# DeepMETv2/DeepMETv2

Hardware: AMD Instinct MI355X
Metric: events/sec (4.5k PF cands, k=16) (higher is better)
Workload: dtype f32

## Files before the change

### deepmetv2_amd/build.py

```python
from __future__ import annotations

import concurrent.futures as cf
import os
import shutil
import subprocess
import sys

PKG_DIR = os.path.dirname(os.path.abspath(__file__))
CSRC = os.path.join(PKG_DIR, "csrc")
OBJ_DIR = os.path.join(CSRC, "_obj")
LIB_PATH = os.path.join(PKG_DIR, "libdmet_hip.so")
SOURCES = ["knn.hip", "radius.hip", "edgeconv.hip", "edgemlp.hip", "misc.hip", "dense.hip", "encoder.hip", "norm.hip", "edgeconv_bwd.hip",
           "head.hip", "finalize.hip", "pool.hip",
           "edgemlp_f32.hip", "edgemlp_bf16.hip", "edgeconv_sum.hip", "gravnet.hip", "attention.hip", "fps.hip"]
HEADERS = [os.path.join(CSRC, h) for h in ("common.h", "knn_common.h", "knn_filter.h", "nls_body.h", "edgemlp_fused.h")] + \
          [os.path.join(PKG_DIR, "..", "include", "dmet.h")]
ARCH = "gfx950"
CXXFLAGS = ["-O3", "-std=c++17", "-fPIC", f"--offload-arch={ARCH}", "-ffp-contract=off", "-Wall",
            "-Wno-unused-function", "-DNDEBUG"]


def _hipcc() -> str:
    exe = shutil.which("hipcc") or "/opt/rocm/bin/hipcc"
    if not os.path.exists(exe):
        raise RuntimeError("hipcc not found: cannot build libdmet_hip.so")
    return exe


def _stale(target: str, deps) -> bool:
    if not os.path.exists(target):
        return True
    t = os.path.getmtime(target)
    return any(os.path.getmtime(d) > t for d in deps if os.path.exists(d))


def _compile(src: str, force: bool) -> str:
    obj = os.path.join(OBJ_DIR, os.path.splitext(src)[0] + ".o")
    path = os.path.join(CSRC, src)
    if force or _stale(obj, [path] + HEADERS):
        cmd = [_hipcc()] + CXXFLAGS + ["-c", path, "-o", obj]
        subprocess.check_call(cmd)
    return obj


def build_hip(force: bool = False, verbose: bool = False) -> str:
    os.makedirs(OBJ_DIR, exist_ok=True)
    with cf.ThreadPoolExecutor(max_workers=min(4, len(SOURCES))) as ex:
        objs = list(ex.map(lambda s: _compile(s, force), SOURCES))
    if force or _stale(LIB_PATH, objs):
        cmd = [_hipcc(), "-shared", "-fPIC", f"--offload-arch={ARCH}", "-o", LIB_PATH] + objs
        if verbose:
            print(" ".join(cmd))
        subprocess.check_call(cmd)
    return LIB_PATH


if __name__ == "__main__":
    print(build_hip(force="--force" in sys.argv, verbose=True))
```

### deepmetv2_amd/csrc/knn.hip

```cpp
#include <stdlib.h>

#include "common.h"
#include "knn_common.h"
#include "nls_body.h"

namespace dmet {
namespace {

constexpr int kTileC = 32;
constexpr int kQMax = 8;
constexpr int kMaxSplit = 8;
constexpr int kWavesPerGroup = 4;

#define DMET_PKSUB_LO " op_sel:[0,0] op_sel_hi:[0,1] neg_lo:[0,1] neg_hi:[0,1]\n\t"
#define DMET_PKSUB_HI " op_sel:[1,0] op_sel_hi:[1,1] neg_lo:[0,1] neg_hi:[0,1]\n\t"
__device__ __forceinline__ void pk_dist_step4(f2 &accA, f2 &accB, f2 vxy, f2 vzw, f2 wxy, f2 wzw, f2 q0, f2 q1, f2 q2,
                                              f2 q3)
{
    f2 t0, t1, t2, t3;
    asm("v_pk_add_f32 %[t0], %[vxy], %[q0]" DMET_PKSUB_LO
        "v_pk_add_f32 %[t1], %[wxy], %[q0]" DMET_PKSUB_LO
        "v_pk_add_f32 %[t2], %[vxy], %[q1]" DMET_PKSUB_HI
        "v_pk_add_f32 %[t3], %[wxy], %[q1]" DMET_PKSUB_HI
        "v_pk_fma_f32 %[a], %[t0], %[t0], %[a]\n\t"
        "v_pk_fma_f32 %[b], %[t1], %[t1], %[b]\n\t"
        "v_pk_add_f32 %[t0], %[vzw], %[q2]" DMET_PKSUB_LO
        "v_pk_add_f32 %[t1], %[wzw], %[q2]" DMET_PKSUB_LO
        "v_pk_fma_f32 %[a], %[t2], %[t2], %[a]\n\t"
        "v_pk_fma_f32 %[b], %[t3], %[t3], %[b]\n\t"
        "v_pk_add_f32 %[t2], %[vzw], %[q3]" DMET_PKSUB_HI
        "v_pk_add_f32 %[t3], %[wzw], %[q3]" DMET_PKSUB_HI
        "v_pk_fma_f32 %[a], %[t0], %[t0], %[a]\n\t"
        "v_pk_fma_f32 %[b], %[t1], %[t1], %[b]\n\t"
        "v_pk_fma_f32 %[a], %[t2], %[t2], %[a]\n\t"
        "v_pk_fma_f32 %[b], %[t3], %[t3], %[b]"
        : [a] "+v"(accA), [b] "+v"(accB), [t0] "=&v"(t0), [t1] "=&v"(t1), [t2] "=&v"(t2), [t3] "=&v"(t3)
        : [vxy] "v"(vxy), [vzw] "v"(vzw), [wxy] "v"(wxy), [wzw] "v"(wzw), [q0] "v"(q0), [q1] "v"(q1), [q2] "v"(q2),
          [q3] "v"(q3));
}

template <bool HI>
__device__ __forceinline__ void pk_sub2(f2 &tA, f2 &tB, f2 v, f2 w, f2 q)
{
    if (HI)
        asm("v_pk_add_f32 %[ta], %[v], %[q]" DMET_PKSUB_HI "v_pk_add_f32 %[tb], %[w], %[q]" DMET_PKSUB_HI
            : [ta] "=&v"(tA), [tb] "=&v"(tB) : [v] "v"(v), [w] "v"(w), [q] "v"(q));
    else
        asm("v_pk_add_f32 %[ta], %[v], %[q]" DMET_PKSUB_LO "v_pk_add_f32 %[tb], %[w], %[q]" DMET_PKSUB_LO
            : [ta] "=&v"(tA), [tb] "=&v"(tB) : [v] "v"(v), [w] "v"(w), [q] "v"(q));
}

__device__ __forceinline__ void pk_fma2(f2 &accA, f2 &accB, f2 tA, f2 tB)
{
    asm("v_pk_fma_f32 %[a], %[ta], %[ta], %[a]\n\t"
        "v_pk_fma_f32 %[b], %[tb], %[tb], %[b]"
        : [a] "+v"(accA), [b] "+v"(accB) : [ta] "v"(tA), [tb] "v"(tB));
}

__device__ __forceinline__ float wrap1(float d, float L)
{
    float a, t;
    asm("v_sub_f32 %[t], %[L], |%[d]|\n\t"
        "v_min_f32 %[a], |%[d]|, %[t]"
        : [a] "=v"(a), [t] "=&v"(t) : [d] "v"(d), [L] "s"(L));
    return a;
}

template <bool HI>
__device__ __forceinline__ void pk_dist_step1_per(f2 &accA, f2 &accB, f2 v, f2 w, f2 q, float L, bool wrap)
{
    f2 tA, tB;
    pk_sub2<HI>(tA, tB, v, w, q);
    if (wrap) {
        tA = f2{wrap1(tA.x, L), wrap1(tA.y, L)};
        tB = f2{wrap1(tB.x, L), wrap1(tB.y, L)};
    }
    pk_fma2(accA, accB, tA, tB);
}

template <int DP, int TQ>
struct KnnShared {
    float4 tile[(kTileC + 1) * DP / 4];
    uint2 queue[TQ][kQMax][kWave];
};

template <int KP>
__device__ __attribute__((noinline)) float drain_queue(const uint2 (*queue)[kWave], int lane, int cnt, bool fresh,
                                                       bool valid, float *__restrict__ ld,
                                                       int32_t *__restrict__ lj)
{
    float d[KP];
    int32_t j[KP];
    if (fresh || !valid) {
#pragma unroll
        for (int p = 0; p < KP; ++p) { d[p] = kKnnSentinel; j[p] = -1; }
    } else {
#pragma unroll
        for (int p = 0; p < KP; p += 4) {
            const float4 v = *reinterpret_cast<const float4 *>(ld + p);
            const int4 w = *reinterpret_cast<const int4 *>(lj + p);
            d[p] = v.x; d[p + 1] = v.y; d[p + 2] = v.z; d[p + 3] = v.w;
            j[p] = w.x; j[p + 1] = w.y; j[p + 2] = w.z; j[p + 3] = w.w;
        }
    }
    int maxcnt = cnt;
#pragma unroll
    for (int off = 32; off > 0; off >>= 1) maxcnt = max(maxcnt, __shfl_xor(maxcnt, off, 64));
    for (int s = 0; s < maxcnt; ++s) {
        if (s < cnt) {
            const uint2 e = queue[s][lane];
            const float nd = __uint_as_float(e.x);
            const int32_t nj = (int32_t)e.y;
            if (nd < d[KP - 1]) {
#pragma unroll
                for (int p = KP - 1; p >= 1; --p) {
                    const bool mq = d[p - 1] > nd;
                    const bool mp = d[p] > nd;
                    const float dn = mq ? d[p - 1] : (mp ? nd : d[p]);
                    const int32_t jn = mq ? j[p - 1] : (mp ? nj : j[p]);
                    d[p] = dn;
                    j[p] = jn;
                }
                if (d[0] > nd) { d[0] = nd; j[0] = nj; }
            }
        }
    }
    if (valid) {
#pragma unroll
        for (int p = 0; p < KP; p += 4) {
            *reinterpret_cast<float4 *>(ld + p) = make_float4(d[p], d[p + 1], d[p + 2], d[p + 3]);
            *reinterpret_cast<int4 *>(lj + p) = make_int4(j[p], j[p + 1], j[p + 2], j[p + 3]);
        }
    }
    return d[KP - 1];
}

#ifdef DMET_KNN_STAMP
__device__ unsigned long long g_knn_stamps[1 << 16][4];
#endif

#ifndef DMET_F2_MIN_NODES
#define DMET_F2_MIN_NODES 800
#endif
constexpr int kF2MinNodes = DMET_F2_MIN_NODES;
constexpr int kFilterMaxSplit = 2;
#ifndef DMET_F2_SPLIT_MIN_NODES
#define DMET_F2_SPLIT_MIN_NODES 2560
#endif
constexpr int kF2SplitMinNodes = DMET_F2_SPLIT_MIN_NODES;
constexpr int kF2MaxNodes = 65536;

struct KnnPlan {
    int total_tiles;
    int n_full;
    int split;
    int form1_events;
// ... 1118 lines not shown
```

### deepmetv2_amd/csrc/knn_filter.h

```cpp
constexpr int kFQ = 64;

typedef float f32x16 __attribute__((ext_vector_type(16)));
typedef short bf16x8 __attribute__((ext_vector_type(8)));
typedef _Float16 f16x8 __attribute__((ext_vector_type(8)));

struct KnnFilterArgs {
    const float *x;
    const int64_t *ptr;
    int B;
    int64_t N;
    int k;
    float *nrm;
    uint8_t *rec;
    const KnnPlan *plan;
    const int32_t *order;
    const int32_t *pos_of;
    const int32_t *tile_ptr;
    float *psd;
    int32_t *psj;
    int32_t *nbr;
    float *dist;
    uint16_t *nbr16;
    int32_t *flags;
    int32_t *any;
// ... 914 lines not shown
        asm volatile("" : "+v"(fq[0]), "+v"(fq[1]));
    }
    float rc = L.rep, rn;
    f32x16 c0 = f2_block<NH>(A, bq[0], fq[0]);
    f32x16 c1 = f2_block<NH>(A, bq[1], fq[1]);
    f32x16 n0, n1;
    f2_load<NH>(A, rec, rbase + min(t_lo + 1, t_hi - 1), lane, hh, rofs);
    float carry = kKnnSentinel;
    if constexpr (NH == 1 && UPD && REC) {
        F2Ops<NH> C;
        f2_load<NH>(B, rec, rbase + min(t_lo + 2, t_hi - 1), lane, hh, rofs);
        for (int t = t_lo; t < t_hi; t += 6) {
            f2_tile<M, UPD, REC, true, NH, false, 3>(L, S, rec, rbase, t, t_hi, c0, c1, n0, n1, rc, rn, A, C, bq, fq, lane, hh,
                                                     alive, carry, rofs);
            if (t + 1 >= t_hi) break;
            f2_tile<M, UPD, REC, true, NH, true, 3>(L, S, rec, rbase, t + 1, t_hi, n0, n1, c0, c1, rn, rc, B, A, bq, fq, lane,
                                                    hh, alive, carry, rofs);
            if (t + 2 >= t_hi) break;
            f2_tile<M, UPD, REC, true, NH, false, 3>(L, S, rec, rbase, t + 2, t_hi, c0, c1, n0, n1, rc, rn, C, B, bq, fq, lane,
                                                     hh, alive, carry, rofs);
            if (t + 3 >= t_hi) break;
            f2_tile<M, UPD, REC, true, NH, true, 3>(L, S, rec, rbase, t + 3, t_hi, n0, n1, c0, c1, rn, rc, A, C, bq, fq, lane,
                                                    hh, alive, carry, rofs);
            if (t + 4 >= t_hi) break;
            f2_tile<M, UPD, REC, true, NH, false, 3>(L, S, rec, rbase, t + 4, t_hi, c0, c1, n0, n1, rc, rn, B, A, bq, fq, lane,
                                                     hh, alive, carry, rofs);
            if (t + 5 >= t_hi) break;
            f2_tile<M, UPD, REC, true, NH, true, 3>(L, S, rec, rbase, t + 5, t_hi, n0, n1, c0, c1, rn, rc, C, B, bq, fq, lane,
                                                    hh, alive, carry, rofs);
        }
        return;
    }
    for (int t = t_lo; t < t_hi; t += 2) {
        f2_tile<M, UPD, REC, true, NH, false>(L, S, rec, rbase, t, t_hi, c0, c1, n0, n1, rc, rn, A, B, bq, fq, lane, hh, alive,
                                              carry, rofs);
        if (t + 1 < t_hi)
            f2_tile<M, UPD, REC, true, NH, true>(L, S, rec, rbase, t + 1, t_hi, n0, n1, c0, c1, rn, rc, B, A, bq, fq, lane, hh,
                                                 alive, carry, rofs);
    }
}

__device__ __forceinline__ int filter_group(const KnnFilterArgs &a)
{
    const int full_groups = a.plan->n_full / kWavesPerGroup;
    return (int)blockIdx.x < full_groups ? xcd_swizzle((int)blockIdx.x, full_groups) : (int)blockIdx.x;
}

template <int KP, int NH = 1>
__device__ __forceinline__ void filter2_wave(const KnnFilterArgs &a, F2Wave &S, int *tickets, int group, int wv, int lane)
{
    constexpr int M = f2_list_len(KP);
    constexpr int D = 32 * NH;
    constexpr int MS = (M + 1 + 3) & ~3;
    const int col = lane & 31, hh = lane >> 5;
    const uint8_t *__restrict__ rec = a.rec;
    const int64_t *__restrict__ ptr = a.ptr;

    const int n_full = a.plan->n_full, split = a.plan->split, total = a.plan->total_tiles;
    const int item = group * kWavesPerGroup + wv;
    int tile = item, sub = 0, nsub = 1;
    if (item >= n_full) {
        const int r = item - n_full;
        tile = n_full + r / split;
        sub = r % split;
        nsub = split;
    }
    if (tile >= total) return;
    const int pos = find_tile_event(a.tile_ptr, a.B, tile);
    const int ev = a.order[pos];
    const int ev_lo = (int)ptr[ev], ev_hi = (int)ptr[ev + 1];
    const int q_first = ev_lo + (tile - a.tile_ptr[pos]) * kFQ;
    if (!f2_in_domain(ev_hi - ev_lo)) {
        if (NH != 1 && sub == 0) {
            const int q = q_first + lane;
            if (q < ev_hi) {
                flag_query(a, q, a.xtile_ptr[pos] + (q - ev_lo) / a.xtile_queries);
            }
        }
        return;
    }
    int clo = ev_lo, chi = ev_hi;
    if (nsub > 1) {
        if (ev_hi - ev_lo < kF2SplitMinNodes) {
            if (sub != 0) return;
            nsub = 1;
        } else {
            const int chunk = (((chi - clo) + nsub - 1) / nsub + 31) & ~31;
            clo = min(chi, clo + sub * chunk);
            chi = min(chi, clo + chunk);
        }
    }
    const int64_t rbase = (ptr[ev] >> 5) + ev;
    const int64_t rlast = rbase + (ev_hi - ev_lo - 1) / 32;
    const int t_lo = (clo - ev_lo) / 32, t_hi = (chi - ev_lo + 31) / 32;

    const int myq = q_first + hh * 32 + col;
    const bool valid = myq < ev_hi;
    float t_fix = -__builtin_inff();
    bool act = valid;
    for (int attempt = 0;; ++attempt) {
    F2Lane<M> L;
#pragma unroll
    for (int p = 0; p < M; ++p) L.tk[p] = kKnnSentinel;
    L.tau = attempt == 0 ? -__builtin_inff() : t_fix;
    L.tq = 0u;
    L.rep = 0.0f;
    L.cnt = 0;
    L.overflow = false;
    {
        f16x8 bq[2][2 * NH];
#pragma unroll
        for (int b = 0; b < 2; ++b) {
            const int64_t qrec = min(rbase + (q_first - ev_lo) / 32 + b, rlast);
            const f16x8 *g = reinterpret_cast<const f16x8 *>(rec + qrec * rec_bytes(NH));
#pragma unroll
            for (int m = 0; m < 2 * NH; ++m) bq[b][m] = g[m * 64 + lane] * (_Float16)-2.0f;
        }
        if (attempt == 0) {
            const int t_def = min(t_hi, t_lo + kF2Defer);
            f2_sweep<M, true, false, NH>(L, S, rec, rbase, t_lo, t_def, bq, lane, hh, valid);
            f2_sweep<M, true, true, NH>(L, S, rec, rbase, t_def, t_hi, bq, lane, hh, valid);
            if (a.cut_scale >= 0.0f) {
                float tkk = kKnnSentinel;
#pragma unroll
                for (int p = 0; p < KP; ++p)
                    if (p == a.k - 1) tkk = L.tk[p];
                if (tkk < kKnnSentinel) {
                    int qi = valid ? myq : ev_lo;
                    asm volatile("" : "+v"(qi));
                    const float cut = f2_cut<NH>(tkk, a.nrm[qi], a.cut_scale);
                    L.tau = fminf(L.tau, cut);
                }
            }
            f2_sweep<M, false, true, NH>(L, S, rec, rbase, t_lo, t_def, bq, lane, hh, valid);
        } else {
            f2_sweep<M, false, true, NH>(L, S, rec, rbase, t_lo, t_hi, bq, lane, hh, valid);
        }
    }
    f2_compact<M>(L, S, lane, kF2Slots);
#if defined(DMET_F2_ABL) && DMET_F2_ABL >= 1
    return;
#endif

    const int64_t qrow_id = valid ? myq : ev_lo;
    float qrow[D];
    {
        const float4 *g = reinterpret_cast<const float4 *>(a.x + qrow_id * D);
#pragma unroll
        for (int c = 0; c < D / 4; ++c) {
            const float4 v = g[c];
            qrow[4 * c] = v.x; qrow[4 * c + 1] = v.y; qrow[4 * c + 2] = v.z; qrow[4 * c + 3] = v.w;
        }
    }
    unsigned long long kk[KP];
#pragma unroll
    for (int p = 0; p < KP; ++p) kk[p] = (unsigned long long)__float_as_uint(kKnnSentinel) << 32;
    const int nent = (act && !L.overflow) ? L.cnt : 0;
    int slot = 0;
    unsigned cmask = 0u;
    int ctile = 0;
    auto pop = [&]() __attribute__((always_inline)) -> int32_t {
        if (cmask == 0u && slot < nent) {
            const uint2 e = S.ent[slot][lane];
            cmask = e.x;
            ctile = (int)(e.y & kF2TileMask);
            ++slot;
        }
        int32_t j = -1;
        if (cmask != 0u) {
            const int r = __builtin_clz(cmask);
            cmask &= ~(0x80000000u >> r);
            j = ev_lo + ctile * 32 + f2_mask_row(r);
        }
        return j;
    };
    const float4 *x4 = reinterpret_cast<const float4 *>(a.x);
#ifdef DMET_RR_PRIO
    __builtin_amdgcn_s_setprio(DMET_RR_PRIO);
#endif
    if constexpr (NH != 1) {
        for (;;) {
            const int32_t j = pop();
            if (!__any(j >= 0)) break;
            const float4 *row = x4 + (int64_t)(j >= 0 ? j : ev_lo) * (D / 4);
            float4 v[D / 4];
#pragma unroll
            for (int c = 0; c < D / 4; ++c) v[c] = row[c];
            float dc = 0.0f;
#pragma unroll
            for (int c = 0; c < D / 4; ++c) {
                float df;
                df = v[c].x - qrow[4 * c + 0]; dc = __builtin_fmaf(df, df, dc);
                df = v[c].y - qrow[4 * c + 1]; dc = __builtin_fmaf(df, df, dc);
                df = v[c].z - qrow[4 * c + 2]; dc = __builtin_fmaf(df, df, dc);
                df = v[c].w - qrow[4 * c + 3]; dc = __builtin_fmaf(df, df, dc);
            }
            const unsigned long long nk =
                j >= 0 ? (((unsigned long long)__float_as_uint(dc) << 32) | (unsigned)j) : ~0ull;
            bool g[KP];
#pragma unroll
            for (int p = 0; p < KP; ++p) g[p] = kk[p] > nk;
#pragma unroll
            for (int p = KP - 1; p >= 1; --p) kk[p] = g[p - 1] ? kk[p - 1] : (g[p] ? nk : kk[p]);
            kk[0] = g[0] ? nk : kk[0];
        }
    } else {
    struct HalfRows { float4 v0, v1, v2, v3, v4, v5, v6, v7; };
#ifdef DMET_RR_FULLROW
    auto fetch = [&](int32_t j) __attribute__((always_inline)) -> HalfRows {
        const int32_t jc = j >= 0 ? j : ev_lo;
        const int64_t o = lane & 7;
        const int sub = lane >> 3;
        HalfRows R;
        R.v0 = x4[(int64_t)__shfl(jc, 0 + sub, 64) * 8 + o];
        R.v1 = x4[(int64_t)__shfl(jc, 8 + sub, 64) * 8 + o];
        R.v2 = x4[(int64_t)__shfl(jc, 16 + sub, 64) * 8 + o];
        R.v3 = x4[(int64_t)__shfl(jc, 24 + sub, 64) * 8 + o];
        R.v4 = x4[(int64_t)__shfl(jc, 32 + sub, 64) * 8 + o];
        R.v5 = x4[(int64_t)__shfl(jc, 40 + sub, 64) * 8 + o];
        R.v6 = x4[(int64_t)__shfl(jc, 48 + sub, 64) * 8 + o];
        R.v7 = x4[(int64_t)__shfl(jc, 56 + sub, 64) * 8 + o];
        return R;
    };
#else
    auto fetch = [&](int32_t j) __attribute__((always_inline)) -> HalfRows {
        const int32_t jc = j >= 0 ? j : ev_lo;
        const int64_t o = 4 * 0 + (lane & 3);
        const int64_t r0 = (int64_t)__shfl(jc, 0 + (lane >> 2), 64) * 8 + o;
        const int64_t r1 = (int64_t)__shfl(jc, 16 + (lane >> 2), 64) * 8 + o;
        const int64_t r2 = (int64_t)__shfl(jc, 32 + (lane >> 2), 64) * 8 + o;
        const int64_t r3 = (int64_t)__shfl(jc, 48 + (lane >> 2), 64) * 8 + o;
        HalfRows R;
        R.v0 = x4[r0]; R.v1 = x4[r1]; R.v2 = x4[r2]; R.v3 = x4[r3];
        R.v4 = x4[r0 + 4]; R.v5 = x4[r1 + 4]; R.v6 = x4[r2 + 4]; R.v7 = x4[r3 + 4];
        return R;
    };
#endif
    auto chain16 = [&](float dc, int h) __attribute__((always_inline)) -> float {
#pragma unroll
        for (int c4 = 0; c4 < 4; ++c4) {
            const float4 v = *reinterpret_cast<const float4 *>(&S.rows[lane][4 * c4]);
            const int f0 = 16 * h + 4 * c4;
            float df;
            df = v.x - qrow[f0 + 0]; dc = __builtin_fmaf(df, df, dc);
            df = v.y - qrow[f0 + 1]; dc = __builtin_fmaf(df, df, dc);
            df = v.z - qrow[f0 + 2]; dc = __builtin_fmaf(df, df, dc);
            df = v.w - qrow[f0 + 3]; dc = __builtin_fmaf(df, df, dc);
        }
        return dc;
    };
    auto round = [&](const HalfRows &R, int32_t j) __attribute__((always_inline)) {
#ifdef DMET_RR_FULLROW
        float4 *dst = reinterpret_cast<float4 *>(&S.rows[lane >> 3][4 * (lane & 3)]);
        constexpr int kS8 = 8 * (kF2RowF + 4) / 4;
        const bool lowhalf = (lane & 4) == 0;
        wave_sync();
        if (lowhalf) {
            dst[0] = R.v0; dst[kS8] = R.v1; dst[2 * kS8] = R.v2; dst[3 * kS8] = R.v3;
            dst[4 * kS8] = R.v4; dst[5 * kS8] = R.v5; dst[6 * kS8] = R.v6; dst[7 * kS8] = R.v7;
        }
        wave_sync();
        float dc = chain16(0.0f, 0);
        wave_sync();
        if (!lowhalf) {
            dst[0] = R.v0; dst[kS8] = R.v1; dst[2 * kS8] = R.v2; dst[3 * kS8] = R.v3;
            dst[4 * kS8] = R.v4; dst[5 * kS8] = R.v5; dst[6 * kS8] = R.v6; dst[7 * kS8] = R.v7;
        }
        wave_sync();
        dc = chain16(dc, 1);
#else
        float4 *dst = reinterpret_cast<float4 *>(&S.rows[lane >> 2][4 * (lane & 3)]);
        constexpr int kStride = 16 * (kF2RowF + 4) / 4;
        wave_sync();
        dst[0] = R.v0; dst[kStride] = R.v1; dst[2 * kStride] = R.v2; dst[3 * kStride] = R.v3;
        wave_sync();
        float dc = chain16(0.0f, 0);
        wave_sync();
        dst[0] = R.v4; dst[kStride] = R.v5; dst[2 * kStride] = R.v6; dst[3 * kStride] = R.v7;
        wave_sync();
        dc = chain16(dc, 1);
#endif
        const unsigned long long nk =
            j >= 0 ? (((unsigned long long)__float_as_uint(dc) << 32) | (unsigned)j) : ~0ull;
        bool g[KP];
#pragma unroll
        for (int p = 0; p < KP; ++p) g[p] = kk[p] > nk;
#pragma unroll
        for (int p = KP - 1; p >= 1; --p) kk[p] = g[p - 1] ? kk[p - 1] : (g[p] ? nk : kk[p]);
        kk[0] = g[0] ? nk : kk[0];
    };
#ifdef DMET_RR_THREE
    constexpr bool kThreeRounds = KP <= 16;
#else
    constexpr bool kThreeRounds = false;
#endif
    if constexpr (kThreeRounds) {
        int32_t ja = pop(), jb, jc;
        HalfRows pa = fetch(ja), pb, pc;
        jb = pop();
        pb = fetch(jb);
        for (;;) {
            if (!__any(ja >= 0)) break;
            jc = pop(); pc = fetch(jc);
            round(pa, ja);
            if (!__any(jb >= 0)) break;
            ja = pop(); pa = fetch(ja);
            round(pb, jb);
            if (!__any(jc >= 0)) break;
            jb = pop(); pb = fetch(jb);
            round(pc, jc);
        }
    } else {
        int32_t ja = pop(), jb;
        HalfRows pa = fetch(ja), pb;
        for (;;) {
            if (!__any(ja >= 0)) break;
            jb = pop(); pb = fetch(jb);
            round(pa, ja);
            if (!__any(jb >= 0)) break;
            ja = pop(); pa = fetch(ja);
            round(pb, jb);
        }
    }
    }
#ifdef DMET_RR_PRIO
    __builtin_amdgcn_s_setprio(0);
#endif
    float kd[KP];
    int32_t kj[KP];
#pragma unroll
    for (int p = 0; p < KP; ++p) {
        kd[p] = __uint_as_float((unsigned)(kk[p] >> 32));
        kj[p] = kd[p] == kKnnSentinel ? -1 : (int32_t)(unsigned)kk[p];
    }
    int elane = lane, eq = myq;
    asm volatile("" : "+v"(elane), "+v"(eq));
    const int k = a.k;
    const float tau = L.tau;
    auto emit = [&](const bool rows_on, const bool coop) __attribute__((always_inline)) -> float {
        float kth = -1.0f;
#pragma unroll
        for (int p = 0; p < KP; ++p)
            if (p == k - 1 && kj[p] >= 0) kth = kd[p];
        if constexpr (KP % 4 == 0 && KP <= 20) {
            if (coop && a.emit_coalesced && k == KP) {
                constexpr int RP = KP / 4;
                const unsigned long long on = __ballot(rows_on);
                unsigned *stg = reinterpret_cast<unsigned *>(&S);
                const int64_t blk = (int64_t)q_first * KP;
                wave_sync();
#pragma unroll
                for (int q = 0; q < RP; ++q)
                    *reinterpret_cast<uint4 *>(stg + elane * KP + 4 * q) =
                        make_uint4((unsigned)kj[4 * q], (unsigned)kj[4 * q + 1], (unsigned)kj[4 * q + 2], (unsigned)kj[4 * q + 3]);
                wave_sync();
#pragma unroll
                for (int t = 0; t < RP; ++t) {
                    const int pi = t * 64 + elane;
                    const uint4 v = *reinterpret_cast<const uint4 *>(stg + 4 * pi);
                    if ((on >> (pi / RP)) & 1ull) *reinterpret_cast<uint4 *>(a.nbr + blk + 4 * pi) = v;
                }
                wave_sync();
#pragma unroll
                for (int q = 0; q < RP; ++q)
                    *reinterpret_cast<uint4 *>(stg + elane * KP + 4 * q) =
                        make_uint4(__float_as_uint(kd[4 * q]), __float_as_uint(kd[4 * q + 1]), __float_as_uint(kd[4 * q + 2]),
                                   __float_as_uint(kd[4 * q + 3]));
                wave_sync();
#pragma unroll
                for (int t = 0; t < RP; ++t) {
                    const int pi = t * 64 + elane;
                    const uint4 v = *reinterpret_cast<const uint4 *>(stg + 4 * pi);
                    if ((on >> (pi / RP)) & 1ull) *reinterpret_cast<uint4 *>(a.dist + blk + 4 * pi) = v;
                }
                if (a.nbr16) {
                    if constexpr (KP % 8 == 0) {
                        constexpr int RH = KP / 8;
                        wave_sync();
#pragma unroll
                        for (int q = 0; q < RH; ++q) {
                            uint4 w;
                            w.x = (unsigned)local_id16(kj[8 * q], ev_lo) | ((unsigned)local_id16(kj[8 * q + 1], ev_lo) << 16);
                            w.y = (unsigned)local_id16(kj[8 * q + 2], ev_lo) | ((unsigned)local_id16(kj[8 * q + 3], ev_lo) << 16);
                            w.z = (unsigned)local_id16(kj[8 * q + 4], ev_lo) | ((unsigned)local_id16(kj[8 * q + 5], ev_lo) << 16);
                            w.w = (unsigned)local_id16(kj[8 * q + 6], ev_lo) | ((unsigned)local_id16(kj[8 * q + 7], ev_lo) << 16);
                            *reinterpret_cast<uint4 *>(stg + elane * (KP / 2) + 4 * q) = w;
                        }
                        wave_sync();
#pragma unroll
                        for (int t = 0; t < RH; ++t) {
                            const int pi = t * 64 + elane;
                            const uint4 v = *reinterpret_cast<const uint4 *>(stg + 4 * pi);
                            if ((on >> (pi / RH)) & 1ull)
                                *reinterpret_cast<uint4 *>(reinterpret_cast<unsigned *>(a.nbr16 + blk) + 4 * pi) = v;
                        }
                    } else if (rows_on) {
                        uint16_t *r16 = a.nbr16 + (int64_t)eq * k;
#pragma unroll
                        for (int p = 0; p + 1 < KP; p += 2)
                            reinterpret_cast<unsigned *>(r16)[p >> 1] =
                                (unsigned)local_id16(kj[p], ev_lo) | ((unsigned)local_id16(kj[p + 1], ev_lo) << 16);
                    }
                }
                wave_sync();
                return kth;
            }
        }
        if (!rows_on) return kth;
#pragma unroll
        for (int p = 0; p < KP; ++p) {
            if (p < k) {
                a.nbr[(int64_t)eq * k + p] = kj[p];
                a.dist[(int64_t)eq * k + p] = kd[p];
            }
        }
        if (a.nbr16) {
            uint16_t *r16 = a.nbr16 + (int64_t)eq * k;
            if ((k & 1) == 0) {
#pragma unroll
                for (int p = 0; p + 1 < KP; p += 2)
                    if (p < k)
                        reinterpret_cast<unsigned *>(r16)[p >> 1] =
                            (unsigned)local_id16(kj[p], ev_lo) | ((unsigned)local_id16(kj[p + 1], ev_lo) << 16);
            } else {
#pragma unroll
                for (int p = 0; p < KP; ++p)
                    if (p < k) r16[p] = local_id16(kj[p], ev_lo);
            }
        }
        return kth;
    };
    if (nsub == 1) {
        bool retry = false;
        const float kth = emit(act, true);
        if (act) {
            const float nx = a.nrm[eq];
            const float an = __builtin_sqrtf(nx) * 1.000001f;
            const float rn = an + __builtin_sqrtf(fmaxf(kth, 0.0f)) * 1.00002f;
            const float slack = f2_slack(an, rn, NH == 1 ? 1.0f : 1.5f);
            const bool wideq = !(nx < kF16WideLimit * kF16WideLimit);
            const bool fail = L.overflow || wideq || (f2_full<NH>(tau) && !(kth >= 0.0f && f2_cert_T<NH>(tau) + nx - slack > kth));
            const float ts = f2_cert_threshold<NH>(kth, nx, slack);
            retry = fail && attempt == 0 && !L.overflow && !wideq && kth >= 0.0f && f2_cert_T<NH>(ts) + nx - slack > kth &&
                    ts < kKnnSentinel;
            if (fail && !retry) {
                flag_query(a, eq, a.xtile_ptr[pos] + (eq - ev_lo) / a.xtile_queries);
#ifdef DMET_KNN_WHY
                a.qflag[eq] = (uint8_t)(1 | (L.overflow ? 2 : 0) | (wideq ? 4 : 0) | (kth < 0.0f ? 8 : 0) | (attempt ? 16 : 0) |
                                         (!(ts < kKnnSentinel) ? 32 : 0) | (!(f2_cert_T<NH>(ts) + nx - slack > kth) ? 64 : 0));
                a.dist[(int64_t)eq * k + 0] = tau; a.dist[(int64_t)eq * k + 1] = kth; a.dist[(int64_t)eq * k + 2] = slack; a.dist[(int64_t)eq * k + 3] = (float)L.cnt;
#endif
            }
            t_fix = retry ? ts : -__builtin_inff();
        }
        if (!__any(retry)) return;
        const int nretry = __popcll(__ballot(retry));
        if (elane == 0) {
            atomicAdd(a.retries, 1);
            atomicAdd(a.retries + 1, nretry);
        }
        act = retry;
        continue;
    }
    static_assert(kFilterMaxSplit == 2 && kWavesPerGroup % 2 == 0, "pairs of sub-sweeps share a workgroup");
    const int64_t fslot = (int64_t)(tile - n_full) * kFQ + hh * 32 + col;
    if (valid) {
        float *ld = a.psd + (fslot * nsub + sub) * MS;
        int32_t *lj = a.psj + (fslot * nsub + sub) * MS;
#pragma unroll
        for (int p = 0; p < KP; ++p) { ld[p] = kd[p]; lj[p] = kj[p]; }
        ld[M] = tau;
        lj[M] = L.overflow ? 1 : 0;
    }
    __builtin_amdgcn_fence(__ATOMIC_RELEASE, "workgroup");
    int arrived = 0;
    if (elane == 0) arrived = atomicAdd(&tickets[wv >> 1], 1);
    arrived = __builtin_amdgcn_readfirstlane(arrived);
    if (arrived == 0) return;
    __builtin_amdgcn_fence(__ATOMIC_ACQUIRE, "workgroup");
    float tau_o = kKnnSentinel;
    int of_o = 0;
    if (valid) {
        const float *ld = a.psd + (fslot * nsub + (sub ^ 1)) * MS;
        const int32_t *lj = a.psj + (fslot * nsub + (sub ^ 1)) * MS;
        tau_o = ld[M];
        of_o = lj[M];
#pragma unroll
        for (int p = 0; p < KP; ++p) {
            const float od = ld[p];
            const int32_t oj = lj[p];
            const unsigned long long nk = oj >= 0 ? (((unsigned long long)__float_as_uint(od) << 32) | (unsigned)oj) : ~0ull;
            bool g[KP];
#pragma unroll
            for (int q = 0; q < KP; ++q) g[q] = kk[q] > nk;
#pragma unroll
            for (int q = KP - 1; q >= 1; --q) kk[q] = g[q - 1] ? kk[q - 1] : (g[q] ? nk : kk[q]);
            kk[0] = g[0] ? nk : kk[0];
        }
#pragma unroll
        for (int p = 0; p < KP; ++p) {
            kd[p] = __uint_as_float((unsigned)(kk[p] >> 32));
            kj[p] = kd[p] == kKnnSentinel ? -1 : (int32_t)(unsigned)kk[p];
        }
        const float kth = emit(true, false);
        const float nx = a.nrm[eq];
        const float an = __builtin_sqrtf(nx) * 1.000001f;
        const float rn = an + __builtin_sqrtf(fmaxf(kth, 0.0f)) * 1.00002f;
        const float slack = f2_slack(an, rn, NH == 1 ? 1.0f : 1.5f);
        const bool wideq = !(nx < kF16WideLimit * kF16WideLimit);
        const bool fail_a = f2_full<NH>(tau) && !(kth >= 0.0f && f2_cert_T<NH>(tau) + nx - slack > kth);
        const bool fail_b = f2_full<NH>(tau_o) && !(kth >= 0.0f && f2_cert_T<NH>(tau_o) + nx - slack > kth);
        if (L.overflow || of_o != 0 || wideq || fail_a || fail_b)
            flag_query(a, eq, a.xtile_ptr[pos] + (eq - ev_lo) / a.xtile_queries);
    }
    return;
    }
}

template <int KP, int NH = 1>
__global__ __launch_bounds__(kWave * kWavesPerGroup, kF2WavesPerSimd) void knn_filter12_kernel(const KnnFilterArgs a)
{
    union WaveLds {
        F2Wave f2;
#ifndef DMET_F2_LEAN
        FilterQueue<filter_queue_len(filter_list_len(KP))> f1;
#endif
    };
    __shared__ WaveLds sh_all[kWavesPerGroup];
    if constexpr (NH == 1) {
        if (a.rP != nullptr && (int)blockIdx.x >= a.first_rider) {
            static_assert(sizeof(WaveLds) >= sizeof(float) * kNlsLdsFloats, "a wavefront's LDS holds the transposition tiles");
            const int rwv = __builtin_amdgcn_readfirstlane(threadIdx.x >> 6);
            const int64_t wave = (int64_t)((int)blockIdx.x - a.first_rider) * kWavesPerGroup + rwv;
            const int64_t nwaves = (int64_t)((int)gridDim.x - a.first_rider) * kWavesPerGroup;
            float *tp = reinterpret_cast<float *>(&sh_all[rwv]);
            if (a.r_sliced == 2)
                node_linear_split_bf16_wave<32, 32>(a.x, a.N, a.rW, a.rb, a.rP, reinterpret_cast<unsigned short *>(a.rQ), wave,
                                                    nwaves, threadIdx.x & 63);
            else if (a.r_sliced == 1) node_linear_split_wave<32, 32, true>(a.x, a.N, a.rW, a.rb, a.rP, a.rQ, tp, wave, nwaves, threadIdx.x & 63);
            else node_linear_split_wave<32, 32, false>(a.x, a.N, a.rW, a.rb, a.rP, a.rQ, tp, wave, nwaves, threadIdx.x & 63);
            return;
        }
    }
    static_assert(sizeof(WaveLds) == sizeof(F2Wave), "the union is sized by the second form");
#ifndef DMET_F2_LEAN
    static_assert(sizeof(FilterQueue<filter_queue_len(filter_list_len(KP))>) <= sizeof(F2Wave) - 8, "ticket bytes are free");
#endif
    static_assert(kWavesPerGroup / 2 <= 2, "two ticket words");
    int *tickets = reinterpret_cast<int *>(&sh_all[0].f2.rows[kF2StageRows - 1][kF2RowF + 2]);
    const int wv = __builtin_amdgcn_readfirstlane(threadIdx.x >> 6), lane = threadIdx.x & 63;
    if (threadIdx.x < kWavesPerGroup / 2) tickets[threadIdx.x] = 0;
    __syncthreads();
    const int group = filter_group(a);
    filter2_wave<KP, NH>(a, sh_all[wv].f2, tickets, group, wv, lane);
#ifndef DMET_F2_LEAN
    if constexpr (NH == 1) filter1_wave<KP>(a, sh_all[wv].f1, group, wv, lane);
#endif
}

template <int KP>
__global__ __launch_bounds__(256) void knn_rerank_kernel(const KnnFilterArgs a)
{
    constexpr int M = filter_list_len(KP);
    constexpr int MS = (M + 1 + 3) & ~3;
    constexpr int QPW = kWave / M;
    constexpr int QPB = 4 * QPW;
    constexpr int EMAX = kFilterMaxSplit * M;
    __shared__ float sc[QPB][EMAX];
    __shared__ int32_t sj[QPB][EMAX];
    __shared__ float skth[QPB];
    __shared__ int sfail[QPB];
    __shared__ float qbuf[QPB][32];
    constexpr int PARTS = (kFQ + QPB - 1) / QPB;
    const int wv = __builtin_amdgcn_readfirstlane(threadIdx.x >> 6), lane = threadIdx.x & 63;
    const int qw = lane / M, l = lane - qw * M;
    const int slot = wv * QPW + min(qw, QPW - 1);
    const int bid = blockIdx.x;
    if (a.form2 && a.plan->form1_events == 0) return;
    const int n_full = a.plan->n_full, split = a.plan->split;
    const int ft = n_full + bid / PARTS, part = bid % PARTS;
    if (ft >= a.plan->total_tiles) return;
    const int pos = find_tile_event(a.tile_ptr, a.B, ft);
    const int ev = a.order[pos];
    const int64_t ev_lo = a.ptr[ev], ev_hi = a.ptr[ev + 1];
    if (a.form2 && f2_in_domain((int)(ev_hi - ev_lo))) return;
    const int qoff = part * QPB + wv * QPW + qw;
    const int64_t q = ev_lo + (int64_t)(ft - a.tile_ptr[pos]) * kFQ + qoff;
    const bool active = qw < QPW && qoff < kFQ && q < ev_hi;
    const int64_t qq = active ? q : ev_lo;
    const int nsub = split;
    const int64_t fslot = (int64_t)(ft - n_full) * kFQ + (active ? qoff : 0);
    const float *bd = a.psd + fslot * nsub * MS;
    const int32_t *bj = a.psj + fslot * nsub * MS;
    const int E = nsub * M;

    int32_t myj[kFilterMaxSplit];
#pragma unroll
    for (int t = 0; t < kFilterMaxSplit; ++t) myj[t] = (active && t < nsub) ? bj[t * MS + l] : -1;
    float vtau = kKnnSentinel, vnx = 0.0f;
    bool voverflow = false;
    if (active && l < nsub) { vtau = bd[l * MS + M]; voverflow = bj[l * MS + M] != 0; vnx = a.nrm[qq]; }
    if (lane < QPW * 8) {
        const int w = lane >> 3;
        const int64_t qrow_id = min(ev_lo + (int64_t)(ft - a.tile_ptr[pos]) * kFQ + part * QPB + wv * QPW + w, ev_hi - 1);
        *reinterpret_cast<float4 *>(&qbuf[wv * QPW + w][4 * (lane & 7)]) =
            reinterpret_cast<const float4 *>(a.x + qrow_id * 32)[lane & 7];
    }
    float myc[kFilterMaxSplit];
    wave_sync();
#pragma unroll 1
    for (int t = 0; t < kFilterMaxSplit; ++t) {
        float ct = kKnnSentinel;
        int32_t j = (t == 0) ? myj[0] : myj[kFilterMaxSplit - 1];
        if (active && t < nsub) {
            const int idx = t * M + l;
            if (j >= 0) {
                const float4 *g = reinterpret_cast<const float4 *>(a.x + (int64_t)j * 32);
                float4 crow[8];
#pragma unroll
                for (int c = 0; c < 8; ++c) crow[c] = g[c];
                float acc = 0.0f;
#pragma unroll
                for (int c = 0; c < 8; ++c) {
                    const float4 v = crow[c];
                    const float4 qv = *reinterpret_cast<const float4 *>(&qbuf[slot][4 * c]);
                    float df;
                    df = v.x - qv.x; acc = __builtin_fmaf(df, df, acc);
                    df = v.y - qv.y; acc = __builtin_fmaf(df, df, acc);
                    df = v.z - qv.z; acc = __builtin_fmaf(df, df, acc);
                    df = v.w - qv.w; acc = __builtin_fmaf(df, df, acc);
                }
                ct = acc;
                if (!(ct < kKnnSentinel)) {
                    ct = kKnnSentinel;
                    j = -1;
                    if (t == 0) myj[0] = -1; else myj[kFilterMaxSplit - 1] = -1;
                }
            }
            sc[slot][idx] = ct;
            sj[slot][idx] = (j >= 0) ? j : (0x7fffffff - idx);
        }
        if (t == 0) myc[0] = ct; else myc[kFilterMaxSplit - 1] = ct;
    }
    if (active && l == 0) { skth[slot] = -1.0f; sfail[slot] = 0; }
    wave_sync();
    const int k = a.k;
#pragma unroll
    for (int t = 0; t < kFilterMaxSplit; ++t) {
        if (active && t < nsub) {
            const int idx = t * M + l;
            const float c = myc[t];
            const int32_t jj = (myj[t] >= 0) ? myj[t] : (0x7fffffff - idx);
            int rank = 0;
            for (int e = 0; e < E; ++e) {
                const float ce = sc[slot][e];
// ... 26 lines not shown
```

Before: 48390.

## Use f64 min/max sorting network for kNN top-k keys and scalar-base fetch

Replaces the 64-bit integer compare-and-select insertion into the top-k list with f64 min/max instructions on the key bits reinterpreted as doubles. Distances are clamped below the sentinel so every key stays a finite positive double that orders the same way as the integer key. Also prefetches the next slot entry in pop with branchless updates. The row fetch now uses a wave-uniform event base pointer with 32-bit local offsets instead of 64-bit per-lane indexing. These changes aim to cut VALU instruction count and address arithmetic in the hot refinement loop, at the cost of relying on the ordering of the bit patterns reinterpreted as doubles.

Measured after the change: 49630, median of 6. +2.6%, better.

```diff
diff --git a/deepmetv2_amd/build.py b/deepmetv2_amd/build.py
--- a/deepmetv2_amd/build.py
+++ b/deepmetv2_amd/build.py
@@ -13,7 +13,8 @@
 SOURCES = ["knn.hip", "radius.hip", "edgeconv.hip", "edgemlp.hip", "misc.hip", "dense.hip", "encoder.hip", "norm.hip", "edgeconv_bwd.hip",
            "head.hip", "finalize.hip", "pool.hip",
            "edgemlp_f32.hip", "edgemlp_bf16.hip", "edgeconv_sum.hip", "gravnet.hip", "attention.hip", "fps.hip"]
-HEADERS = [os.path.join(CSRC, h) for h in ("common.h", "knn_common.h", "knn_filter.h", "nls_body.h", "edgemlp_fused.h")] + \
+HEADERS = [os.path.join(CSRC, h) for h in ("common.h", "knn_common.h", "knn_filter.h", "knn_key64.h", "nls_body.h",
+                                           "edgemlp_fused.h")] + \
           [os.path.join(PKG_DIR, "..", "include", "dmet.h")]
 ARCH = "gfx950"
 CXXFLAGS = ["-O3", "-std=c++17", "-fPIC", f"--offload-arch={ARCH}", "-ffp-contract=off", "-Wall",
diff --git a/deepmetv2_amd/csrc/knn.hip b/deepmetv2_amd/csrc/knn.hip
--- a/deepmetv2_amd/csrc/knn.hip
+++ b/deepmetv2_amd/csrc/knn.hip
@@ -2,6 +2,7 @@
 
 #include "common.h"
 #include "knn_common.h"
+#include "knn_key64.h"
 #include "nls_body.h"
 
 namespace dmet {
diff --git a/deepmetv2_amd/csrc/knn_filter.h b/deepmetv2_amd/csrc/knn_filter.h
--- a/deepmetv2_amd/csrc/knn_filter.h
+++ b/deepmetv2_amd/csrc/knn_filter.h
@@ -1090,27 +1090,28 @@
             qrow[4 * c] = v.x; qrow[4 * c + 1] = v.y; qrow[4 * c + 2] = v.z; qrow[4 * c + 3] = v.w;
         }
     }
-    unsigned long long kk[KP];
-#pragma unroll
-    for (int p = 0; p < KP; ++p) kk[p] = (unsigned long long)__float_as_uint(kKnnSentinel) << 32;
+    static_assert(__builtin_bit_cast(unsigned, kKnnSentinel) == kKey64SentinelBits, "knn_key64.h clamps to the sentinel");
+    double kk[KP];
+#pragma unroll
+    for (int p = 0; p < KP; ++p) kk[p] = key64_as_double(kKey64Empty);
     const int nent = (act && !L.overflow) ? L.cnt : 0;
     int slot = 0;
     unsigned cmask = 0u;
     int ctile = 0;
+    uint2 enext = S.ent[0][lane];
     auto pop = [&]() __attribute__((always_inline)) -> int32_t {
-        if (cmask == 0u && slot < nent) {
-            const uint2 e = S.ent[slot][lane];
-            cmask = e.x;
-            ctile = (int)(e.y & kF2TileMask);
-            ++slot;
-        }
-        int32_t j = -1;
+        const bool take = cmask == 0u && slot < nent;
+        cmask = take ? enext.x : cmask;
+        ctile = take ? (int)(enext.y & kF2TileMask) : ctile;
+        slot += take ? 1 : 0;
+        enext = S.ent[min(slot, kF2Slots - 1)][lane];
+        int32_t jl = -1;
         if (cmask != 0u) {
             const int r = __builtin_clz(cmask);
             cmask &= ~(0x80000000u >> r);
-            j = ev_lo + ctile * 32 + f2_mask_row(r);
-        }
-        return j;
+            jl = ctile * 32 + f2_mask_row(r);
+        }
+        return jl;
     };
     const float4 *x4 = reinterpret_cast<const float4 *>(a.x);
 #ifdef DMET_RR_PRIO
@@ -1118,9 +1119,10 @@
 #endif
     if constexpr (NH != 1) {
         for (;;) {
-            const int32_t j = pop();
-            if (!__any(j >= 0)) break;
-            const float4 *row = x4 + (int64_t)(j >= 0 ? j : ev_lo) * (D / 4);
+            const int32_t jl = pop();
+            if (!__any(jl >= 0)) break;
+            const int32_t j = ev_lo + jl;
+            const float4 *row = x4 + (int64_t)(jl >= 0 ? j : ev_lo) * (D / 4);
             float4 v[D / 4];
 #pragma unroll
             for (int c = 0; c < D / 4; ++c) v[c] = row[c];
@@ -1133,20 +1135,13 @@
                 df = v[c].z - qrow[4 * c + 2]; dc = __builtin_fmaf(df, df, dc);
                 df = v[c].w - qrow[4 * c + 3]; dc = __builtin_fmaf(df, df, dc);
             }
-            const unsigned long long nk =
-                j >= 0 ? (((unsigned long long)__float_as_uint(dc) << 32) | (unsigned)j) : ~0ull;
-            bool g[KP];
-#pragma unroll
-            for (int p = 0; p < KP; ++p) g[p] = kk[p] > nk;
-#pragma unroll
-            for (int p = KP - 1; p >= 1; --p) kk[p] = g[p - 1] ? kk[p - 1] : (g[p] ? nk : kk[p]);
-            kk[0] = g[0] ? nk : kk[0];
+            key64_insert<KP>(kk, key64_word(__float_as_uint(dc), (unsigned)j, jl >= 0));
         }
     } else {
     struct HalfRows { float4 v0, v1, v2, v3, v4, v5, v6, v7; };
 #ifdef DMET_RR_FULLROW
-    auto fetch = [&](int32_t j) __attribute__((always_inline)) -> HalfRows {
-        const int32_t jc = j >= 0 ? j : ev_lo;
+    auto fetch = [&](int32_t jl) __attribute__((always_inline)) -> HalfRows {
+        const int32_t jc = ev_lo + (jl >= 0 ? jl : 0);
         const int64_t o = lane & 7;
         const int sub = lane >> 3;
         HalfRows R;
@@ -1161,16 +1156,25 @@
         return R;
     };
 #else
-    auto fetch = [&](int32_t j) __attribute__((always_inline)) -> HalfRows {
-        const int32_t jc = j >= 0 ? j : ev_lo;
-        const int64_t o = 4 * 0 + (lane & 3);
-        const int64_t r0 = (int64_t)__shfl(jc, 0 + (lane >> 2), 64) * 8 + o;
-        const int64_t r1 = (int64_t)__shfl(jc, 16 + (lane >> 2), 64) * 8 + o;
-        const int64_t r2 = (int64_t)__shfl(jc, 32 + (lane >> 2), 64) * 8 + o;
-        const int64_t r3 = (int64_t)__shfl(jc, 48 + (lane >> 2), 64) * 8 + o;
+    const uint64_t xb = reinterpret_cast<uint64_t>(a.x + (int64_t)ev_lo * D);
+    const uint64_t xbs = ((uint64_t)(unsigned)__builtin_amdgcn_readfirstlane((int)(xb >> 32)) << 32) |
+                         (unsigned)__builtin_amdgcn_readfirstlane((int)xb);
+    typedef float f32x4 __attribute__((ext_vector_type(4)));
+    typedef const f32x4 __attribute__((address_space(1))) *GlobalRow;
+    auto ld = [](GlobalRow g, int i) __attribute__((always_inline)) -> float4 {
+        const f32x4 v = g[i];
+        return make_float4(v.x, v.y, v.z, v.w);
+    };
+    auto fetch = [&](int32_t jl) __attribute__((always_inline)) -> HalfRows {
+        const int32_t jc = jl >= 0 ? jl : 0;
+        const unsigned o = 16u * (lane & 3);
+        const GlobalRow r0 = (GlobalRow)(xbs + (uint64_t)(((unsigned)__shfl(jc, 0 + (lane >> 2), 64) << 7) + o));
+        const GlobalRow r1 = (GlobalRow)(xbs + (uint64_t)(((unsigned)__shfl(jc, 16 + (lane >> 2), 64) << 7) + o));
+        const GlobalRow r2 = (GlobalRow)(xbs + (uint64_t)(((unsigned)__shfl(jc, 32 + (lane >> 2), 64) << 7) + o));
+        const GlobalRow r3 = (GlobalRow)(xbs + (uint64_t)(((unsigned)__shfl(jc, 48 + (lane >> 2), 64) << 7) + o));
         HalfRows R;
-        R.v0 = x4[r0]; R.v1 = x4[r1]; R.v2 = x4[r2]; R.v3 = x4[r3];
-        R.v4 = x4[r0 + 4]; R.v5 = x4[r1 + 4]; R.v6 = x4[r2 + 4]; R.v7 = x4[r3 + 4];
+        R.v0 = ld(r0, 0); R.v1 = ld(r1, 0); R.v2 = ld(r2, 0); R.v3 = ld(r3, 0);
+        R.v4 = ld(r0, 4); R.v5 = ld(r1, 4); R.v6 = ld(r2, 4); R.v7 = ld(r3, 4);
         return R;
     };
 #endif
@@ -1187,7 +1191,7 @@
         }
         return dc;
     };
-    auto round = [&](const HalfRows &R, int32_t j) __attribute__((always_inline)) {
+    auto round = [&](const HalfRows &R, int32_t jl) __attribute__((always_inline)) {
 #ifdef DMET_RR_FULLROW
         float4 *dst = reinterpret_cast<float4 *>(&S.rows[lane >> 3][4 * (lane & 3)]);
         constexpr int kS8 = 8 * (kF2RowF + 4) / 4;
@@ -1218,14 +1222,7 @@
         wave_sync();
         dc = chain16(dc, 1);
 #endif
-        const unsigned long long nk =
-            j >= 0 ? (((unsigned long long)__float_as_uint(dc) << 32) | (unsigned)j) : ~0ull;
-        bool g[KP];
-#pragma unroll
-        for (int p = 0; p < KP; ++p) g[p] = kk[p] > nk;
-#pragma unroll
-        for (int p = KP - 1; p >= 1; --p) kk[p] = g[p - 1] ? kk[p - 1] : (g[p] ? nk : kk[p]);
-        kk[0] = g[0] ? nk : kk[0];
+        key64_insert<KP>(kk, key64_word(__float_as_uint(dc), (unsigned)(ev_lo + jl), jl >= 0));
     };
 #ifdef DMET_RR_THREE
     constexpr bool kThreeRounds = KP <= 16;
@@ -1268,8 +1265,8 @@
     int32_t kj[KP];
 #pragma unroll
     for (int p = 0; p < KP; ++p) {
-        kd[p] = __uint_as_float((unsigned)(kk[p] >> 32));
-        kj[p] = kd[p] == kKnnSentinel ? -1 : (int32_t)(unsigned)kk[p];
+        kd[p] = __uint_as_float((unsigned)(key64_as_word(kk[p]) >> 32));
+        kj[p] = kd[p] == kKnnSentinel ? -1 : (int32_t)(unsigned)key64_as_word(kk[p]);
     }
     int elane = lane, eq = myq;
     asm volatile("" : "+v"(elane), "+v"(eq));
@@ -1427,18 +1424,12 @@
         for (int p = 0; p < KP; ++p) {
             const float od = ld[p];
             const int32_t oj = lj[p];
-            const unsigned long long nk = oj >= 0 ? (((unsigned long long)__float_as_uint(od) << 32) | (unsigned)oj) : ~0ull;
-            bool g[KP];
-#pragma unroll
-            for (int q = 0; q < KP; ++q) g[q] = kk[q] > nk;
-#pragma unroll
-            for (int q = KP - 1; q >= 1; --q) kk[q] = g[q - 1] ? kk[q - 1] : (g[q] ? nk : kk[q]);
-            kk[0] = g[0] ? nk : kk[0];
+            key64_insert<KP>(kk, key64_word(__float_as_uint(od), (unsigned)oj, oj >= 0));
         }
 #pragma unroll
         for (int p = 0; p < KP; ++p) {
-            kd[p] = __uint_as_float((unsigned)(kk[p] >> 32));
-            kj[p] = kd[p] == kKnnSentinel ? -1 : (int32_t)(unsigned)kk[p];
+            kd[p] = __uint_as_float((unsigned)(key64_as_word(kk[p]) >> 32));
+            kj[p] = kd[p] == kKnnSentinel ? -1 : (int32_t)(unsigned)key64_as_word(kk[p]);
         }
         const float kth = emit(true, false);
         const float nx = a.nrm[eq];
diff --git a/deepmetv2_amd/csrc/knn_key64.h b/deepmetv2_amd/csrc/knn_key64.h
--- /dev/null
+++ b/deepmetv2_amd/csrc/knn_key64.h
@@ -0,0 +1,62 @@
+#pragma once
+#include <stdint.h>
+#include <string.h>
+#if !defined(__HIP_DEVICE_COMPILE__)
+#include <math.h>
+#endif
+
+#if defined(__HIPCC__)
+#define DMET_KEY64_FN __host__ __device__ __forceinline__
+#else
+#define DMET_KEY64_FN inline
+#endif
+
+namespace dmet {
+
+constexpr unsigned kKey64SentinelBits = 0x501502F9u;
+constexpr unsigned long long kKey64Empty = (unsigned long long)kKey64SentinelBits << 32;
+
+DMET_KEY64_FN unsigned long long key64_word(unsigned dbits, unsigned j)
+{
+    const unsigned hi = dbits < kKey64SentinelBits ? dbits : kKey64SentinelBits;
+    return ((unsigned long long)hi << 32) | j;
+}
+
+DMET_KEY64_FN unsigned long long key64_word(unsigned dbits, unsigned j, bool live)
+{
+    return key64_word(live ? dbits : 0xFFFFFFFFu, j);
+}
+
+DMET_KEY64_FN double key64_as_double(unsigned long long w)
+{
+    double d;
+    memcpy(&d, &w, 8);
+    return d;
+}
+
+DMET_KEY64_FN unsigned long long key64_as_word(double d)
+{
+    unsigned long long w;
+    memcpy(&w, &d, 8);
+    return w;
+}
+
+template <int KP>
+DMET_KEY64_FN void key64_insert(double (&kk)[KP], unsigned long long w)
+{
+    const double nk = key64_as_double(w);
+#if defined(__HIP_DEVICE_COMPILE__)
+#pragma unroll
+    for (int p = KP - 1; p >= 1; --p) {
+        double t;
+        asm("v_min_f64 %0, %1, %2" : "=v"(t) : "v"(kk[p]), "v"(nk));
+        asm("v_max_f64 %0, %1, %2" : "=v"(kk[p]) : "v"(kk[p - 1]), "v"(t));
+    }
+    asm("v_min_f64 %0, %1, %2" : "=v"(kk[0]) : "v"(kk[0]), "v"(nk));
+#else
+    for (int p = KP - 1; p >= 1; --p) kk[p] = fmax(kk[p - 1], fmin(kk[p], nk));
+    kk[0] = fmin(kk[0], nk);
+#endif
+}
+
+}
```
